# posgraph/coupe.DVSG

Hardware: AMD Instinct MI355X
Metric: stabilized frames/sec (1280x720 RGB) (higher is better)
Workload: dtype f32

## Files before the change

### coupe/dvsg_amd/_lib.py

```python
import ctypes
import os

_HERE = os.path.dirname(os.path.abspath(__file__))
LIB_PATH = os.environ.get("DVSG_AMD_LIB") or os.path.join(_HERE, "libdvsg_amd.so")
ABI_VERSION = 1

c_float_p = ctypes.POINTER(ctypes.c_float)
_vp = ctypes.c_void_p
_i = ctypes.c_int

SIGNATURES = {
    "dvsg_tps_solve_f32": [_vp, _vp, _i, _i, _i, _vp, _vp],
    "dvsg_tps_solve_checked_f32": [_vp, _vp, _i, _i, _i, _vp, _vp, _vp],
    "dvsg_tps_warp_f32": [_vp, _vp, _vp, _i, _i, _i, _i, _i, _i, _i, _vp, _vp, _vp, _vp],
    "dvsg_flow_warp_f32": [_vp, _vp, _i, _i, _i, _i, _vp, _vp],
    "dvsg_stn_sample_f32": [_vp, _vp, _vp, _i, _i, _i, _i, _i, _i, _vp, _vp],
    "dvsg_grid_affine_f32": [_vp, _vp, _i, _i, _i, _i, _i, _i, _vp, _vp, _vp, _vp],
    "dvsg_grid_projective_f32": [_vp, _vp, _i, _i, _i, _i, _i, _i, _vp, _vp, _vp, _vp],
    "dvsg_elastic_constants_f32": [_i, _vp, _vp],
    "dvsg_grid_elastic_f32": [_vp, _vp, _vp, _i, _vp, _i, _i, _i, _i, _i, _i, _vp, _vp, _vp, _vp],
    "dvsg_scale_rgb_f32": [_vp, _i, _i, _i, _i, _vp, _vp],
    "dvsg_locnet_create": [_i, ctypes.POINTER(ctypes.c_char_p), ctypes.POINTER(_vp),
                           ctypes.POINTER(_i), ctypes.POINTER(ctypes.c_int64), ctypes.POINTER(_vp)],
    "dvsg_locnet_destroy": [_vp],
# ... 99 lines not shown


def load():
    global _lib
    if _lib is not None:
        return _lib
    if not os.path.isfile(LIB_PATH):
        raise DvsgError(
            "libdvsg_amd.so not found at %s: build it with ./build.sh (hipcc --offload-arch=gfx950). "
            "coupe.dvsg_amd has no CPU or PyTorch fallback." % LIB_PATH)
    lib = ctypes.CDLL(LIB_PATH)
    lib.dvsg_abi_version.restype = ctypes.c_int
    lib.dvsg_last_error_string.restype = ctypes.c_char_p
    lib.dvsg_target_arch.restype = ctypes.c_char_p
    if lib.dvsg_abi_version() != ABI_VERSION:
        raise DvsgError("libdvsg_amd.so ABI %d != expected %d" % (lib.dvsg_abi_version(), ABI_VERSION))
    for name, argtypes in SIGNATURES.items():
        fn = getattr(lib, name)
        fn.argtypes = argtypes
        fn.restype = ctypes.c_int
    _lib = lib
    for env, opt in (("DVSG_CONV_VARIANT", b"conv_variant"), ("DVSG_FUSE_CONV", b"fuse_conv"),
                     ("DVSG_F16_SPLIT", b"f16_split"), ("DVSG_FUSE_SHORTCUT", b"fuse_shortcut"),
                     ("DVSG_CONV1_VARIANT", b"conv1_variant"), ("DVSG_F16_PAIR_MASK", b"f16_pair_mask"),
                     ("DVSG_WIDE16_PACKED", b"wide16_packed"), ("DVSG_WIDE16_AROWS", b"wide16_arows"),
                     ("DVSG_WIDE16_HREUSE", b"wide16_hreuse"), ("DVSG_FUSED_HREUSE", b"fused_hreuse"),
                     ("DVSG_CONCAT_SC", b"concat_sc"), ("DVSG_FLOW_TILED", b"flow_tiled")):
        if os.environ.get(env) and os.environ.get("DVSG_DEBUG") == "1":
            check(lib.dvsg_debug_set_option(opt, int(os.environ[env])), "dvsg_debug_set_option")
    return lib


def check(status, what):
    if status != 0:
        msg = load().dvsg_last_error_string().decode("utf-8", "replace")
        raise DvsgError("%s failed (status %d): %s" % (what, status, msg))


def call(name, *args):
    check(getattr(load(), name)(*args), name)
```

### coupe/dvsg_amd/csrc/cnn_kernels.h

```cpp
#pragma once
#include <type_traits>

#include "common.h"

namespace dvsg {

enum Precision { kF32 = 0, kF16 = 1, kF32S = 2, kF32X = 3 };
constexpr size_t elem_size(int prec) { return prec == kF16 ? 2 : 4; }
enum ConvMath { kMathF32, kMathF32S, kMathF32X, kMathF16Pairs, kMathF16Plain };
constexpr Precision storage_of(ConvMath m) { return m == kMathF32S ? kF32S : m == kMathF16Pairs || m == kMathF16Plain ? kF16 : kF32; }
constexpr ConvMath math_of(int prec, bool pairs) {
  return prec == kF16 ? (pairs ? kMathF16Pairs : kMathF16Plain) : prec == kF32S ? kMathF32S : prec == kF32X ? kMathF32X : kMathF32;
}
constexpr size_t elem_size(ConvMath m) { return elem_size((int)storage_of(m)); }
static_assert(storage_of(kMathF32) == kF32 && storage_of(kMathF32X) == kF32 && storage_of(kMathF32S) == kF32S &&
              storage_of(kMathF16Pairs) == kF16 && storage_of(kMathF16Plain) == kF16, "ConvMath -> storage format");
static_assert(math_of(kF32, false) == kMathF32 && math_of(kF32, true) == kMathF32 && math_of(kF32S, false) == kMathF32S &&
              math_of(kF32S, true) == kMathF32S && math_of(kF32X, false) == kMathF32X && math_of(kF32X, true) == kMathF32X &&
              math_of(kF16, true) == kMathF16Pairs && math_of(kF16, false) == kMathF16Plain, "(Precision, pairs) -> ConvMath");
static_assert(elem_size(kMathF32) == 4 && elem_size(kMathF32S) == 4 && elem_size(kMathF32X) == 4 &&
              elem_size(kMathF16Pairs) == 2 && elem_size(kMathF16Plain) == 2, "ConvMath -> bytes per tensor element");

struct ConvWeights {
  const void *rows = nullptr, *packed = nullptr, *packed_a = nullptr, *packed_h = nullptr;
// ... 90 lines not shown
constexpr int kSrcAligned = 1;
constexpr int kSrcKindShift = 1;
constexpr int kSrcMasked = 8;
constexpr int conv1_src(int kind, bool aligned, bool masked) {
  return (kind << kSrcKindShift) | (aligned ? kSrcAligned : 0) | (masked ? kSrcMasked : 0);
}
struct Conv1Src {
  const void *base;
  const int *table;
  int n_pool;
  const float *mask = nullptr;
};
struct Conv1Weights {
  const float *f32;
  const _Float16 *f16;
  const _Float16 *pieces;
  const unsigned short *x3;
  const float *bias;
};
int launch_conv1(int out_prec, const Conv1Src &src, int src_kind, const Conv1Weights &wt, void *y, int B, int H, int W, int Ho,
                 int Wo, int cin, hipStream_t s);
int prepare_rootconv();
int prepare_root_band();

int launch_maxpool(int prec, const void *x, void *y, int B, int H, int W, int C, int Ho, int Wo, int pad_top,
                   int pad_left, hipStream_t s);

constexpr int kPoolSplits = 8;
int launch_avgpool_partial(int prec, const void *x, float *part, int B, int HW, int C, hipStream_t s);

int launch_f16_to_f32(const void *x, float *y, size_t n, hipStream_t s);
int launch_p_to_f32(const void *x, float *y, size_t n, hipStream_t s);
int launch_f32_to_p(const float *x, void *y, size_t n, hipStream_t s);

constexpr int kDenseSplits = 8;
int launch_dense(const float *xin, int s_in, const float *bias_in, float scale_in, int lrelu_in,
                 const float *W, float *out_part, int B, int K, int N, hipStream_t s);
int launch_dense_finalize(const float *part, int s_in, float scale, const float *bias, float *out, int B,
                          int N, hipStream_t s);

}
```

### coupe/dvsg_amd/csrc/common.h

```cpp
#pragma once
#include <hip/hip_runtime.h>

#include <cstdarg>
#include <cstdio>

#include "../../../include/dvsg_amd.h"

namespace dvsg {

char *error_buffer();
int fail(int status, const char *fmt, ...) __attribute__((format(printf, 2, 3)));

inline hipStream_t as_stream(void *s) { return reinterpret_cast<hipStream_t>(s); }

inline int check_launch(const char *what) {
  hipError_t e = hipGetLastError();
  if (e != hipSuccess) return fail(DVSG_ERR_HIP, "%s: %s", what, hipGetErrorString(e));
  return DVSG_OK;
}

#define DVSG_REQUIRE(cond, ...)                                  \
  do {                                                           \
    if (!(cond)) return ::dvsg::fail(DVSG_ERR_INVALID_ARG, __VA_ARGS__); \
  } while (0)
// ... 26 lines not shown
int tps_render_impl(const double *winv_cols, const float *coord, const float *F_t, const uint8_t *src, int B, int H, int W,
                    int P, int channel_flip, float *T, float *out_f32, uint8_t *out_u8, int u8_W, int u8_x0, void *stream,
                    const float *zoom = nullptr, int render_filter = DVSG_RENDER_BILINEAR ,
                    int render_border = DVSG_BORDER_BLACK ,
                    RenderShape shape = RenderShape() );
int tps_render_nv12_check(const float *F_t, const uint8_t *y, const uint8_t *uv, size_t pitch, size_t frame_stride, int n,
                          int H, int W, const float *T, const uint8_t *out_y, const uint8_t *out_uv, size_t out_pitch,
                          size_t out_frame_stride, const char *fn = "dvsg_tps_render_nv12");
int tps_render_p010_check(const uint8_t *y, const uint8_t *uv, size_t pitch, size_t frame_stride, int n, int W,
                          const uint8_t *out_y, const uint8_t *out_uv, size_t out_pitch, size_t out_frame_stride, const char *fn);
int tps_render_nv12_impl(const double *winv_cols, const float *coord, const float *F_t, const uint8_t *y, const uint8_t *uv,
                         size_t pitch, size_t frame_stride, int n, int H, int W, int P, float *T, uint8_t *out_y,
                         uint8_t *out_uv, size_t out_pitch, size_t out_frame_stride, void *stream,
                         const float *zoom = nullptr, int render_filter = DVSG_RENDER_BILINEAR,
                         int render_border = DVSG_BORDER_BLACK, RenderShape shape = RenderShape(),
                         int surface_format = DVSG_SURFACE_NV12);
int tps_coverage_impl(const char *fn, const float *coord, long coord_bstride, const float *T, const float *zoom, int B, int P,
                      int src_H, int src_W, int out_h, int out_w, int32_t *n_border, int32_t *key_min, void *workspace,
                      size_t workspace_bytes, void *stream);

struct DebugOptions {
  int conv_variant = 0;
  int conv1_variant = 0;
  int wide16_min_tiles = 128;
  int wide16_packed = 1;
  int wide16_arows = 1;
  int wide16_hreuse = 1;
  int fused_hreuse = 1;
  int fuse_conv = 1;
  int fuse_shortcut = 1;
  int concat_sc = 1;
  int x3_conv1 = 1;
  int x3_fuse = 3;
  int f16_split = 1;
  int f16_pair_mask = 0xFFFF;
  int flow_tiled = 1;
  int flow_rounds = 4;
  int warp_xcd = 0;
};
extern DebugOptions g_opt;

inline int ceil_div(long a, long b) { return (int)((a + b - 1) / b); }

__device__ __forceinline__ uint8_t to_u8(double x) {
  const double d = x * 255.0;
  return d >= 255.0 ? (uint8_t)255 : (d > 0.0 ? (uint8_t)(int)d : (uint8_t)0);
// ... 36 lines not shown
```

### coupe/dvsg_amd/csrc/conv1_pool.hip

```cpp
#include <cstdint>
#include <type_traits>
#include <utility>

#include "cnn_device.h"
#include "cnn_kernels.h"

namespace dvsg {
namespace {

constexpr int C1_TILE = 128;
constexpr int C1_SEG_PAD = 5488;
constexpr int C1_WELEMS = 64 * kConv1Ld;
constexpr int C1_LDC = 68;

template <int NT, int GROUPS, bool ALIGNED, bool MASKED = false>
struct Conv1Row {
  static constexpr bool kRing = false;
  typedef float floatx4_u __attribute__((ext_vector_type(4), aligned(4)));
  floatx4 nmean[GROUPS];
  long idx[GROUPS];
  unsigned col_ok, full;
  bool fast;
  struct Data {
    floatx4 reg[GROUPS];
// ... 448 lines not shown
  __syncthreads();
  TO *yrow = y + (((size_t)b * Ho + ho) * Wo + wo0) * 64 + 4 * (tid & 15);
  conv1_tile_out<NT / 16>(Cs, conv1_tile_bias(bias, tid), tid, wo0, Wo,
                          [&](int row, float4 v) __attribute__((always_inline)) { store4(yrow + (size_t)row * 64, v); });
#ifdef DVSG_STAMPS
  if (tid == 0 && blockIdx.x < 65536) {
    unsigned long long *o = g_c1_stamps + (size_t)blockIdx.x * 8;
    const unsigned long long t_end = C1_STAMP();
    o[0] = st[0]; o[1] = st[1]; o[2] = st[2]; o[3] = st[3]; o[4] = st[4];
    o[5] = t_loop_end - t_begin;
    o[6] = t_end - t_begin;
    o[7] = __builtin_amdgcn_s_memrealtime() - r_begin;
  }
#endif
}

constexpr int RB_NT = 512;
constexpr int RB_IN4 = (C1_SEG_PAD / 4 + RB_NT - 1) / RB_NT;
constexpr int RB_WLOADS = (C1_WELEMS / 4 + RB_NT - 1) / RB_NT;
constexpr int RB_SLOTS = 3;
constexpr size_t RB_LDS = sizeof(float) * (size_t)(2 * C1_WELEMS + RB_SLOTS * C1_SEG_PAD);
static_assert(RB_LDS <= 160 * 1024, "the band kernel's LDS must fit a CU");

template <int SRC>
__global__ __launch_bounds__(RB_NT) __attribute__((amdgpu_waves_per_eu(2, 2)))
void root_band_kernel(const Conv1Src src, const float *__restrict__ wt1, const float *__restrict__ bias,
                      float *__restrict__ y, int H, int W, int Ho, int Wo, int wtiles, int bands, int ppb, int nbig) {
  constexpr int NT = RB_NT, MI = 2;
  static_assert(C1_TILE * C1_LDC <= C1_WELEMS, "epilogue tile must fit in a weight buffer");
  extern __shared__ __attribute__((aligned(16))) float rb_lds[];
  float *const w_s = rb_lds;
  float *const in_s = rb_lds + 2 * C1_WELEMS;
  const int tid = threadIdx.x;
  const int lane = tid & 63, wave = tid >> 6;
  const int wr = wave >> 2, wm = (wave >> 1) & 1, wn = wave & 1;
  const int r = lane & 31, h = lane >> 5;

  const Conv1Tile tile = conv1_tile(wtiles, bands);
  const int b = tile.b, band = tile.ho, wo0 = tile.wo0;
  const int pairs = (Ho + 1) / 2;
  const int p0 = band * ppb - (band > nbig ? band - nbig : 0);
  const int p1 = min(p0 + (band < nbig ? ppb : ppb - 1), pairs);
  if (p0 >= p1) return;

#ifdef DVSG_STAMPS
  unsigned long long st[8] = {0, 0, 0, 0, 0, 0, 0, 0};
  const unsigned long long t_begin = C1_STAMP(), r_begin = __builtin_amdgcn_s_memrealtime();
#endif
  typedef typename Conv1RowSel<NT, RB_IN4, SRC>::type Row;
  Row row;
  row.init(src, tid, b, wo0, H, W, C1_SEG_PAD);
  if constexpr (Row::kRing) {
    for (int e = tid; e < RB_SLOTS * C1_SEG_PAD; e += NT) in_s[e] = 0.f;
    __syncthreads();
  }
  typename Row::Data rd[3];
  floatx4 w_reg[RB_WLOADS];
  auto load_w = [&](int kh) __attribute__((always_inline)) {
    const floatx4 *wsrc = reinterpret_cast<const floatx4 *>(wt1 + (size_t)kh * C1_WELEMS);
#pragma unroll
    for (int i = 0; i < RB_WLOADS; ++i) {
      const int q = tid + NT * i;
      w_reg[i] = wsrc[q < C1_WELEMS / 4 ? q : 0];
    }
  };
  auto put_w = [&](int i, float *dst) __attribute__((always_inline)) {
    const int q = tid + NT * i;
    if (q < C1_WELEMS / 4) reinterpret_cast<floatx4 *>(dst)[q] = w_reg[i];
  };
  auto put_row = [&](const typename Row::Data &d, float *slot) __attribute__((always_inline)) {
    if constexpr (Row::kRing) {
      row.scatter(d, [&](int e, float v) __attribute__((always_inline)) { slot[e] = v; });
    } else {
#pragma unroll
      for (int i = 0; i < RB_IN4; ++i) {
        const int q = tid + NT * i;
        const floatx4 v = row.scaled(d, i);
        if (q < C1_SEG_PAD / 4) reinterpret_cast<floatx4 *>(slot)[q] = v;
      }
    }
  };
  auto load_first = [&](int ho_) __attribute__((always_inline)) {
#pragma unroll
    for (int i = 0; i < 3; ++i) row.load(rd[i], 2 * ho_ - 3 + i);
    load_w(0);
  };
#ifdef DVSG_STAMPS
  st[0] = C1_STAMP() - t_begin;
#endif
  load_first(2 * p0);

  for (int p = p0; p < p1; ++p) {
    const int ho = 2 * p;
#ifdef DVSG_STAMPS
    const unsigned long long f0 = C1_STAMP();
#endif
#pragma unroll
    for (int i = 0; i < RB_WLOADS; ++i) put_w(i, w_s);
#pragma unroll
    for (int i = 0; i < 3; ++i) {
      __builtin_amdgcn_sched_barrier(0);
      put_row(rd[i], in_s + i * C1_SEG_PAD);
    }
    __builtin_amdgcn_sched_barrier(0);
    floatx16 acc[MI], acc2[MI];
#pragma unroll
    for (int mi = 0; mi < MI; ++mi)
#pragma unroll
      for (int q = 0; q < 16; ++q) acc[mi][q] = acc2[mi][q] = 0.f;
#ifdef DVSG_STAMPS
    const unsigned long long f1 = C1_STAMP();
    __syncthreads();
    st[2] += f1 - f0;
    st[3] += C1_STAMP() - f1;
#else
    __syncthreads();
#endif

    int s_up = 0;
    for (int t = 0; t < 7; ++t) {
#ifdef DVSG_STAMPS
      const unsigned long long s3 = C1_STAMP();
#endif
      if (t < 6) {
        row.load(rd[0], 2 * ho + t);
        load_w(t + 1);
      }
#ifdef DVSG_STAMPS
      st[4] += C1_STAMP() - s3;
#endif
      __builtin_amdgcn_sched_barrier(0);
      const int s_lo = s_up == 0 ? 2 : s_up - 1;
      const float *a0 = in_s + (wr ? s_lo : s_up) * C1_SEG_PAD + 2 * kConv1Cin * (wm * 32 * MI + r) + 2 * h;
      const float *bp = w_s + (t & 1) * C1_WELEMS + (wn * 32 + r) * kConv1Ld + 2 * h;
      float *w_next = w_s + ((t + 1) & 1) * C1_WELEMS;
      constexpr int STEPS = kConv1Kpad / 4, PAIRS = (STEPS + 1) / 2;
      constexpr int WPUT0 = PAIRS / 2;
      float2 va[2][2][MI], vb[2][2];
      auto read_pair = [&](int slot, int g) __attribute__((always_inline)) {
#pragma unroll
        for (int j = 0; j < 2; ++j) {
          if (2 * g + j >= STEPS) break;
#pragma unroll
          for (int mi = 0; mi < MI; ++mi)
            va[slot][j][mi] = *reinterpret_cast<const float2 *>(a0 + mi * (2 * kConv1Cin * 32) + 4 * (2 * g + j));
          vb[slot][j] = *reinterpret_cast<const float2 *>(bp + 4 * (2 * g + j));
        }
      };
      read_pair(0, 0);
#pragma unroll
      for (int g = 0; g < PAIRS; ++g) {
        if (g + 1 < PAIRS) read_pair((g + 1) & 1, g + 1);
        if (g >= WPUT0 && g < WPUT0 + RB_WLOADS) put_w(g - WPUT0, w_next);
        __builtin_amdgcn_sched_barrier(0);
#pragma unroll
        for (int j = 0; j < 2; ++j) {
          if (2 * g + j >= STEPS) break;
#pragma unroll
          for (int mi = 0; mi < MI; ++mi) acc[mi] = mfma32(va[g & 1][j][mi].x, vb[g & 1][j].x, acc[mi]);
#pragma unroll
          for (int mi = 0; mi < MI; ++mi) acc2[mi] = mfma32(va[g & 1][j][mi].y, vb[g & 1][j].y, acc2[mi]);
        }
        __builtin_amdgcn_sched_barrier(0);
      }
      if (t < 6) {
#ifdef DVSG_STAMPS
        const unsigned long long s0 = C1_STAMP();
        __syncthreads();
        const unsigned long long s1 = C1_STAMP();
        put_row(rd[0], in_s + s_up * C1_SEG_PAD);
        const unsigned long long s2 = C1_STAMP();
        __syncthreads();
        st[1] += s1 - s0;
        st[2] += s2 - s1;
        st[3] += C1_STAMP() - s2;
#else
        __syncthreads();
        put_row(rd[0], in_s + s_up * C1_SEG_PAD);
        __syncthreads();
#endif
      }
      s_up = s_up == 2 ? 0 : s_up + 1;
    }

#ifdef DVSG_STAMPS
    const unsigned long long e0 = C1_STAMP();
#endif
    __syncthreads();
    float *Cs = w_s + wr * C1_WELEMS;
#pragma unroll
    for (int mi = 0; mi < MI; ++mi)
      C1_TILE_PUT(Cs, wm * 32 * MI + mi * 32, wn * 32, acc[mi][q] + acc2[mi][q]);
    __builtin_amdgcn_sched_barrier(0);
    if (p + 1 < p1) load_first(ho + 2);
    int tid_e = tid;
    asm volatile("" : "+v"(tid_e));
    const float4 b4 = conv1_tile_bias(bias, tid_e);
    __builtin_amdgcn_sched_barrier(0);
    __syncthreads();
#pragma unroll
    for (int j = 0; j < 2; ++j) {
      if (ho + j >= Ho) break;
      float *yrow = y + (((size_t)b * Ho + ho + j) * Wo + wo0) * 64 + 4 * (tid_e & 15);
      conv1_tile_out<NT / 16>(w_s + j * C1_WELEMS, b4, tid_e, wo0, Wo,
                              [&](int row_, float4 v) __attribute__((always_inline)) { store4(yrow + (size_t)row_ * 64, v); });
    }
    __syncthreads();
#ifdef DVSG_STAMPS
    st[5] += C1_STAMP() - e0;
#endif
  }
#ifdef DVSG_STAMPS
  if (tid == 0 && blockIdx.x < 65536) {
    unsigned long long *o = g_c1_stamps + (size_t)blockIdx.x * 8;
    o[0] = st[0]; o[1] = st[1]; o[2] = st[2]; o[3] = st[3]; o[4] = st[4]; o[5] = st[5];
    o[6] = C1_STAMP() - t_begin;
    o[7] = __builtin_amdgcn_s_memrealtime() - r_begin;
  }
#endif
}

struct PPieces {};

constexpr int rootconv_seg(int cin) { return C1_RING_PX * rootconv_pitch(cin) + 4; }
constexpr int rootconv_wstage(int cin) { return 64 * rootconv_ld(cin) > C1_TILE * C1_LDC ? 64 * rootconv_ld(cin) : C1_TILE * C1_LDC; }
constexpr size_t rootconv_lds_bytes(int cin) { return sizeof(float) * (size_t)(rootconv_wstage(cin) + rootconv_seg(cin)); }
static_assert(rootconv_lds_bytes(3 * kRootMaxFrames) <= 160 * 1024, "the largest window must fit one workgroup's LDS");

template <typename TO, int SRC>
__global__ __launch_bounds__(256)
void rootconv_kernel(const Conv1Src src, const float *__restrict__ wt1, const float *__restrict__ bias, void *__restrict__ y,
                     int H, int W, int Ho, int Wo, int wtiles, int cin) {
  constexpr int NT = 256, MI = 2;
  constexpr int kKind = SRC >> kSrcKindShift & 3;
  constexpr bool kMasked = (SRC & kSrcMasked) != 0;
  static_assert(SRC >= 0 && SRC < 16 && kKind <= kSrcRingU8, "no such conv1 source");
  extern __shared__ __attribute__((aligned(16))) float rc_lds[];
  const int S = cin / 3, pitch = rootconv_pitch(cin), ldw = rootconv_ld(cin), steps = rootconv_kpad(cin) / 4;
  const int welems = 64 * ldw, seg = rootconv_seg(cin);
  float *w_s = rc_lds;
  float *in_s = rc_lds + rootconv_wstage(cin);
  const int tid = threadIdx.x;
// ... 1228 lines not shown
int prepare_rootconv() {
  const int bytes = (int)rootconv_lds_bytes(3 * kRootMaxFrames);
  hipError_t err = hipSuccess;
  auto raise = [&](const void *fn) {
    const hipError_t e = hipFuncSetAttribute(fn, hipFuncAttributeMaxDynamicSharedMemorySize, bytes);
    if (err == hipSuccess) err = e;
  };
  for (int src = 0; src < 16; ++src)
    with_conv1_src<true>(src, [&](auto src_c) {
      constexpr int S = decltype(src_c)::value;
      raise(reinterpret_cast<const void *>(&rootconv_kernel<float, S>));
      raise(reinterpret_cast<const void *>(&rootconv_kernel<_Float16, S>));
      raise(reinterpret_cast<const void *>(&rootconv_kernel<PPieces, S>));
    });
  DVSG_HIP(err);
  return DVSG_OK;
}

int prepare_root_band() {
  hipError_t err = hipSuccess;
  for (int src = 0; src < 16; ++src)
    with_conv1_src<false>(src, [&](auto src_c) {
      constexpr int S = decltype(src_c)::value;
      const hipError_t e = hipFuncSetAttribute(reinterpret_cast<const void *>(&root_band_kernel<S>),
                                               hipFuncAttributeMaxDynamicSharedMemorySize, (int)RB_LDS);
      if (err == hipSuccess) err = e;
    });
  DVSG_HIP(err);
  return DVSG_OK;
}

#ifdef DVSG_STAMPS
extern "C" int dvsg_debug_read_conv1_stamps(void *host, size_t bytes) {
  return hipMemcpyFromSymbol(host, HIP_SYMBOL(g_c1_stamps), bytes) == hipSuccess ? 0 : -3;
}
#endif

int launch_maxpool(int prec, const void *x, void *y, int B, int H, int W, int C, int Ho, int Wo, int pad_top,
                   int pad_left, hipStream_t s) {
  DVSG_REQUIRE(C % 4 == 0 && (prec != kF32S || C % 32 == 0), "maxpool: C=%d must be a multiple of 4 (32 in the f32s format)", C);
  const size_t total = (size_t)B * Ho * Wo * (C / 4);
  const size_t want = (total + 255) / 256;
  DVSG_REQUIRE(want < (1u << 31), "maxpool: %zu blocks do not fit a grid", want);
  const int blocks = (int)want;
  ProfScope prof(kClsMaxpool, s, 0.0, (double)elem_size(prec) * C * ((double)B * H * W + (double)B * Ho * Wo));
  g_last_root_kernel[kRootMaxpool] = prec == kF32S ? 3 : (prec == kF16 ? (C % 8 == 0 ? 2 : 1) : 0);
  if (prec == kF32S)
    hipLaunchKernelGGL(maxpool_p_kernel, dim3(blocks), dim3(256), 0, s, x, y, H, W, C / 4, Ho, Wo, pad_top, pad_left, total);
  else if (prec == kF16 && C % 8 == 0) {
    const size_t total8 = total / 2;
    hipLaunchKernelGGL(maxpool_h8_kernel, dim3((unsigned)((total8 + 255) / 256)), dim3(256), 0, s, static_cast<const _Float16 *>(x),
                       static_cast<_Float16 *>(y), H, W, C / 8, Ho, Wo, pad_top, pad_left, total8);
// ... 11 lines not shown
```

### coupe/dvsg_amd/csrc/locnet.hip

```cpp
#include <atomic>
#include <cmath>
#include <cstring>
#include <map>
#include <string>
#include <vector>

#include "cnn_kernels.h"

namespace dvsg {
namespace {

constexpr float kBnEps = 1e-5f;
const char *kPrefix = "stabNet/localizationNet/";

struct HostArray {
  const float *data;
  int nd;
  int64_t dims[4];
  size_t size() const {
    size_t n = 1;
    for (int i = 0; i < nd; ++i) n *= (size_t)dims[i];
    return n;
  }
};
// ... 420 lines not shown
    } else if (act == kF32S) {
      if (int rc = launch_p_to_f32(x, act_out, n, s)) return rc;
    } else {
      DVSG_HIP(hipMemcpyAsync(act_out, x, n * sizeof(float), hipMemcpyDeviceToDevice, s));
    }
    act_dims[0] = h; act_dims[1] = w; act_dims[2] = c;
    return 1;
  };
#define DVSG_TAP(stage, x, h, w, c)            \
  do {                                         \
    int t_ = tap(stage, x, h, w, c);           \
    if (t_ < 0) return t_;                     \
    if (t_ > 0) return DVSG_OK;                \
  } while (0)
#define DVSG_RUN(call)             \
  do {                             \
    if (int rc_ = (call)) return rc_; \
  } while (0)

  DVSG_RUN(launch_zero_tickets(ws.splitk_counters, (size_t)kMaxConvLaunches * kSplitKMaxTiles, s));
  ConvScratch scratch{ws};
  const bool fuse_allowed = g_opt.fuse_conv != 0 && calib == nullptr;
  reset_root_kernel();
  {
  MarkerRange mr("dvsg/conv1");
  DVSG_RUN(launch_conv1(precision == kF32X && g_opt.x3_conv1 ? kF32X : act, src, src_kind, net->conv1.conv1_images(), ws.bufA, B, H, W,
                        d.H1, d.W1, net->c_in, s));
  }
  DVSG_TAP(0, ws.bufA, d.H1, d.W1, 64);
  {
  MarkerRange mr("dvsg/pool1");
  DVSG_RUN(launch_maxpool(act, ws.bufA, ws.bufB, B, d.H1, d.W1, 64, d.Hp, d.Wp, d.pad_top, d.pad_left, s));
  }
  DVSG_TAP(1, ws.bufB, d.Hp, d.Wp, 64);

  char *X = ws.bufB, *Y = ws.bufA;
  int h = d.Hp, w = d.Wp;
  int stage = 2;
  int unit_in_block = 0, last_block = -1;
  for (const Unit &u : net->units) {
    unit_in_block = u.block == last_block ? unit_in_block + 1 : 1;
    last_block = u.block;
    char range_name[40];
    std::snprintf(range_name, sizeof(range_name), "dvsg/block%d/unit_%d", u.block + 1, unit_in_block);
    MarkerRange mr(range_name);
    const int ho = (h - 1) / u.stride + 1, wo = (w - 1) / u.stride + 1;
    ConvRes res{X, h, w, u.stride};
    auto math = [&](int kind) { return math_of(precision, f16_pairs(net, u.block, kind)); };
    const int calib_slot = 3 * (stage - 2);
    DVSG_RUN(calib_record(calib, calib_slot, X, (long)B * h * w, u.c1.cin, s));
    const bool x3_fused = precision == kF32X && g_opt.x3_fuse == 3;
    const bool x3_unfused = precision == kF32X && (g_opt.x3_fuse == 0 || (g_opt.x3_fuse == 1 && !u.has_shortcut));
    const bool fuse23 = fuse_allowed && !x3_unfused && conv_fusable(act, u.c2.cin, u.c2.cout, u.c3.cout, u.c2.ksize) &&
                        (act != kF16 || (f16_pairs(net, u.block, kKindC2) && f16_pairs(net, u.block, kKindC3) &&
                                         (!u.has_shortcut || f16_pairs(net, u.block, kKindSc))));
// ... 189 lines not shown
  f.B = B; f.H = H; f.W = W; f.Cin = Cin; f.Cout = Cout;
  f.Ho = (H - 1) / stride + 1; f.Wo = (W - 1) / stride + 1;
  f.stride = stride;
  f.res_H = (f.Ho - 1) * res_stride + 1; f.res_W = (f.Wo - 1) * res_stride + 1; f.res_stride = res_stride;
  if (sc_x) {
    f.res = nullptr;
    f.sc_x = sc_x; f.sc_wt = sc_wt; f.sc_bias = sc_bias;
    f.sc_cin = sc_cin;
  }
  return launch_conv3x3_1x1(f, as_stream(stream));
}

int opt_any(int v) { return v; }
int opt_flag(int v) { return v != 0; }
int opt_positive(int v) { return v > 0 ? v : 1; }
int opt_mask16(int v) { return v & 0xFFFF; }
constexpr struct {
  const char *name;
  int DebugOptions::*member;
  int (*normalise)(int);
} kDebugOptions[] = {
    {"conv_variant", &DebugOptions::conv_variant, opt_any},
    {"conv1_variant", &DebugOptions::conv1_variant, opt_any},
    {"wide16_min_tiles", &DebugOptions::wide16_min_tiles, opt_any},
    {"wide16_packed", &DebugOptions::wide16_packed, opt_any},
    {"wide16_arows", &DebugOptions::wide16_arows, opt_any},
    {"wide16_hreuse", &DebugOptions::wide16_hreuse, opt_any},
    {"fused_hreuse", &DebugOptions::fused_hreuse, opt_any},
    {"fuse_conv", &DebugOptions::fuse_conv, opt_any},
    {"fuse_shortcut", &DebugOptions::fuse_shortcut, opt_flag},
    {"concat_sc", &DebugOptions::concat_sc, opt_flag},
    {"x3_conv1", &DebugOptions::x3_conv1, opt_any},
    {"x3_fuse", &DebugOptions::x3_fuse, opt_any},
    {"f16_split", &DebugOptions::f16_split, opt_flag},
    {"f16_pair_mask", &DebugOptions::f16_pair_mask, opt_mask16},
    {"flow_tiled", &DebugOptions::flow_tiled, opt_any},
    {"flow_rounds", &DebugOptions::flow_rounds, opt_positive},
    {"warp_xcd", &DebugOptions::warp_xcd, opt_flag},
};

}
}

extern "C" {

int dvsg_locnet_create(int n_arrays, const char *const *names, const float *const *host_data, const int *ndims,
// ... 652 lines not shown
```

Before: 753.2.

## Fuse root conv1 with 3x3/s2 maxpool in band kernel, fix seams separately

Adds a pooled variant of the root band conv kernel that applies bias+ReLU and a 3x3 stride-2 max-pool in the epilogue. Each block carries the previous row pair in LDS and writes pooled output directly. Partial maxima at tile and band boundaries go to a seam buffer, and a small follow-up kernel merges them. This avoids writing and re-reading the full-resolution 64-channel conv1 activation and drops the separate maxpool pass. The cost is extra LDS, seam traffic and one more launch. It only applies to the f32, even-size, unmasked case.

After: 759.9, median of 6. No clear change (+0.9%).

```diff
diff --git a/coupe/dvsg_amd/_lib.py b/coupe/dvsg_amd/_lib.py
--- a/coupe/dvsg_amd/_lib.py
+++ b/coupe/dvsg_amd/_lib.py
@@ -145,7 +145,8 @@
     _lib = lib
     for env, opt in (("DVSG_CONV_VARIANT", b"conv_variant"), ("DVSG_FUSE_CONV", b"fuse_conv"),
                      ("DVSG_F16_SPLIT", b"f16_split"), ("DVSG_FUSE_SHORTCUT", b"fuse_shortcut"),
-                     ("DVSG_CONV1_VARIANT", b"conv1_variant"), ("DVSG_F16_PAIR_MASK", b"f16_pair_mask"),
+                     ("DVSG_CONV1_VARIANT", b"conv1_variant"), ("DVSG_ROOT_POOL", b"root_pool"),
+                     ("DVSG_F16_PAIR_MASK", b"f16_pair_mask"),
                      ("DVSG_WIDE16_PACKED", b"wide16_packed"), ("DVSG_WIDE16_AROWS", b"wide16_arows"),
                      ("DVSG_WIDE16_HREUSE", b"wide16_hreuse"), ("DVSG_FUSED_HREUSE", b"fused_hreuse"),
                      ("DVSG_CONCAT_SC", b"concat_sc"), ("DVSG_FLOW_TILED", b"flow_tiled")):
diff --git a/coupe/dvsg_amd/csrc/cnn_kernels.h b/coupe/dvsg_amd/csrc/cnn_kernels.h
--- a/coupe/dvsg_amd/csrc/cnn_kernels.h
+++ b/coupe/dvsg_amd/csrc/cnn_kernels.h
@@ -136,6 +136,10 @@
                  int Wo, int cin, hipStream_t s);
 int prepare_rootconv();
 int prepare_root_band();
+bool root_pool_selected(int out_prec, const Conv1Src &src, int B, int Ho, int Wo, int cin);
+int launch_conv1_pooled(const Conv1Src &src, int src_kind, const Conv1Weights &wt, float *pooled, float *seam, int B, int H,
+                        int W, int Ho, int Wo, hipStream_t s);
+int launch_root_pool_seam(float *pooled, const float *seam, int B, int Ho, int Wo, hipStream_t s);
 
 int launch_maxpool(int prec, const void *x, void *y, int B, int H, int W, int C, int Ho, int Wo, int pad_top,
                    int pad_left, hipStream_t s);
diff --git a/coupe/dvsg_amd/csrc/common.h b/coupe/dvsg_amd/csrc/common.h
--- a/coupe/dvsg_amd/csrc/common.h
+++ b/coupe/dvsg_amd/csrc/common.h
@@ -72,6 +72,7 @@
 struct DebugOptions {
   int conv_variant = 0;
   int conv1_variant = 0;
+  int root_pool = 0;
   int wide16_min_tiles = 128;
   int wide16_packed = 1;
   int wide16_arows = 1;
diff --git a/coupe/dvsg_amd/csrc/conv1_pool.hip b/coupe/dvsg_amd/csrc/conv1_pool.hip
--- a/coupe/dvsg_amd/csrc/conv1_pool.hip
+++ b/coupe/dvsg_amd/csrc/conv1_pool.hip
@@ -494,202 +494,80 @@
 constexpr size_t RB_LDS = sizeof(float) * (size_t)(2 * C1_WELEMS + RB_SLOTS * C1_SEG_PAD);
 static_assert(RB_LDS <= 160 * 1024, "the band kernel's LDS must fit a CU");
 
+constexpr int RB_CARRY = (C1_TILE / 2) * 64;
+constexpr size_t RB_POOL_LDS = RB_LDS + sizeof(float) * (size_t)RB_CARRY;
+static_assert(RB_POOL_LDS <= 160 * 1024, "the pooled band kernel's LDS must fit a CU");
+__host__ __device__ constexpr size_t root_pool_colseam_floats(int B, int Ho, int wtiles) { return (size_t)B * Ho * (wtiles - 1) * 64; }
+__host__ __device__ constexpr int root_band_first(int band, int ppb, int nbig) { return band * ppb - (band > nbig ? band - nbig : 0); }
+
 template <int SRC>
 __global__ __launch_bounds__(RB_NT) __attribute__((amdgpu_waves_per_eu(2, 2)))
 void root_band_kernel(const Conv1Src src, const float *__restrict__ wt1, const float *__restrict__ bias,
                       float *__restrict__ y, int H, int W, int Ho, int Wo, int wtiles, int bands, int ppb, int nbig) {
-  constexpr int NT = RB_NT, MI = 2;
-  static_assert(C1_TILE * C1_LDC <= C1_WELEMS, "epilogue tile must fit in a weight buffer");
-  extern __shared__ __attribute__((aligned(16))) float rb_lds[];
-  float *const w_s = rb_lds;
-  float *const in_s = rb_lds + 2 * C1_WELEMS;
-  const int tid = threadIdx.x;
-  const int lane = tid & 63, wave = tid >> 6;
-  const int wr = wave >> 2, wm = (wave >> 1) & 1, wn = wave & 1;
-  const int r = lane & 31, h = lane >> 5;
-
-  const Conv1Tile tile = conv1_tile(wtiles, bands);
-  const int b = tile.b, band = tile.ho, wo0 = tile.wo0;
-  const int pairs = (Ho + 1) / 2;
-  const int p0 = band * ppb - (band > nbig ? band - nbig : 0);
-  const int p1 = min(p0 + (band < nbig ? ppb : ppb - 1), pairs);
-  if (p0 >= p1) return;
-
-#ifdef DVSG_STAMPS
-  unsigned long long st[8] = {0, 0, 0, 0, 0, 0, 0, 0};
-  const unsigned long long t_begin = C1_STAMP(), r_begin = __builtin_amdgcn_s_memrealtime();
-#endif
-  typedef typename Conv1RowSel<NT, RB_IN4, SRC>::type Row;
-  Row row;
-  row.init(src, tid, b, wo0, H, W, C1_SEG_PAD);
-  if constexpr (Row::kRing) {
-    for (int e = tid; e < RB_SLOTS * C1_SEG_PAD; e += NT) in_s[e] = 0.f;
-    __syncthreads();
-  }
-  typename Row::Data rd[3];
-  floatx4 w_reg[RB_WLOADS];
-  auto load_w = [&](int kh) __attribute__((always_inline)) {
-    const floatx4 *wsrc = reinterpret_cast<const floatx4 *>(wt1 + (size_t)kh * C1_WELEMS);
-#pragma unroll
-    for (int i = 0; i < RB_WLOADS; ++i) {
-      const int q = tid + NT * i;
-      w_reg[i] = wsrc[q < C1_WELEMS / 4 ? q : 0];
-    }
+#define RB_POOL 0
+#include "root_band_body.inc"
+#undef RB_POOL
+}
+
+template <int SRC>
+__global__ __launch_bounds__(RB_NT) __attribute__((amdgpu_waves_per_eu(2, 2)))
+void root_band_pool_kernel(const Conv1Src src, const float *__restrict__ wt1, const float *__restrict__ bias,
+                           float *__restrict__ y, float *__restrict__ seam, int H, int W, int Ho, int Wo, int wtiles,
+                           int bands, int ppb, int nbig) {
+#define RB_POOL 1
+#include "root_band_body.inc"
+#undef RB_POOL
+}
+
+__global__ __launch_bounds__(256)
+void root_pool_seam_kernel(float *__restrict__ y, const float *__restrict__ seam, int B, int Ho, int Wo, int wtiles, int bands,
+                           int ppb, int nbig, size_t n_row, size_t n_col) {
+  size_t e = (size_t)blockIdx.x * 256 + threadIdx.x;
+  if (e >= n_row + n_col) return;
+  const int Hp = Ho >> 1, Wp = Wo >> 1;
+  const float *colseam = seam, *rowseam = seam + root_pool_colseam_floats(B, Ho, wtiles);
+  auto max4 = [](float4 a, const float4 c) __attribute__((always_inline)) {
+    a.x = fmaxf(a.x, c.x);
+    a.y = fmaxf(a.y, c.y);
+    a.z = fmaxf(a.z, c.z);
+    a.w = fmaxf(a.w, c.w);
+    return a;
   };
-  auto put_w = [&](int i, float *dst) __attribute__((always_inline)) {
-    const int q = tid + NT * i;
-    if (q < C1_WELEMS / 4) reinterpret_cast<floatx4 *>(dst)[q] = w_reg[i];
-  };
-  auto put_row = [&](const typename Row::Data &d, float *slot) __attribute__((always_inline)) {
-    if constexpr (Row::kRing) {
-      row.scatter(d, [&](int e, float v) __attribute__((always_inline)) { slot[e] = v; });
-    } else {
-#pragma unroll
-      for (int i = 0; i < RB_IN4; ++i) {
-        const int q = tid + NT * i;
-        const floatx4 v = row.scaled(d, i);
-        if (q < C1_SEG_PAD / 4) reinterpret_cast<floatx4 *>(slot)[q] = v;
-      }
-    }
-  };
-  auto load_first = [&](int ho_) __attribute__((always_inline)) {
-#pragma unroll
-    for (int i = 0; i < 3; ++i) row.load(rd[i], 2 * ho_ - 3 + i);
-    load_w(0);
-  };
-#ifdef DVSG_STAMPS
-  st[0] = C1_STAMP() - t_begin;
-#endif
-  load_first(2 * p0);
-
-  for (int p = p0; p < p1; ++p) {
-    const int ho = 2 * p;
-#ifdef DVSG_STAMPS
-    const unsigned long long f0 = C1_STAMP();
-#endif
-#pragma unroll
-    for (int i = 0; i < RB_WLOADS; ++i) put_w(i, w_s);
+  int c4, pc, pr, t = -1;
+  size_t b;
+  float4 m;
+  if (e < n_row) {
+    c4 = (int)(e % 16);
+    e /= 16;
+    pc = (int)(e % Wp);
+    e /= Wp;
+    const int k = (int)(e % (bands - 1));
+    b = e / (bands - 1);
+    pr = root_band_first(k + 1, ppb, nbig) - 1;
+    m = load4(y + (((b * Hp + pr) * Wp + pc) * 64 + 4 * c4));
+    m = max4(m, load4(rowseam + (((b * (bands - 1) + k) * Wp + pc) * 64 + 4 * c4)));
+    if (pc % (C1_TILE / 2) == C1_TILE / 2 - 1 && pc + 1 < Wp) t = pc / (C1_TILE / 2);
+  } else {
+    e -= n_row;
+    c4 = (int)(e % 16);
+    e /= 16;
+    t = (int)(e % (wtiles - 1));
+    e /= wtiles - 1;
+    pr = (int)(e % Hp);
+    b = e / Hp;
+    pc = (C1_TILE / 2) * (t + 1) - 1;
+    const int band = pr < nbig * ppb ? pr / ppb : nbig + (pr - nbig * ppb) / (ppb > 1 ? ppb - 1 : 1);
+    if (band + 1 < bands && root_band_first(band + 1, ppb, nbig) == pr + 1) return;
+    m = load4(y + (((b * Hp + pr) * Wp + pc) * 64 + 4 * c4));
+  }
+  if (t >= 0) {
 #pragma unroll
     for (int i = 0; i < 3; ++i) {
-      __builtin_amdgcn_sched_barrier(0);
-      put_row(rd[i], in_s + i * C1_SEG_PAD);
-    }
-    __builtin_amdgcn_sched_barrier(0);
-    floatx16 acc[MI], acc2[MI];
-#pragma unroll
-    for (int mi = 0; mi < MI; ++mi)
-#pragma unroll
-      for (int q = 0; q < 16; ++q) acc[mi][q] = acc2[mi][q] = 0.f;
-#ifdef DVSG_STAMPS
-    const unsigned long long f1 = C1_STAMP();
-    __syncthreads();
-    st[2] += f1 - f0;
-    st[3] += C1_STAMP() - f1;
-#else
-    __syncthreads();
-#endif
-
-    int s_up = 0;
-    for (int t = 0; t < 7; ++t) {
-#ifdef DVSG_STAMPS
-      const unsigned long long s3 = C1_STAMP();
-#endif
-      if (t < 6) {
-        row.load(rd[0], 2 * ho + t);
-        load_w(t + 1);
-      }
-#ifdef DVSG_STAMPS
-      st[4] += C1_STAMP() - s3;
-#endif
-      __builtin_amdgcn_sched_barrier(0);
-      const int s_lo = s_up == 0 ? 2 : s_up - 1;
-      const float *a0 = in_s + (wr ? s_lo : s_up) * C1_SEG_PAD + 2 * kConv1Cin * (wm * 32 * MI + r) + 2 * h;
-      const float *bp = w_s + (t & 1) * C1_WELEMS + (wn * 32 + r) * kConv1Ld + 2 * h;
-      float *w_next = w_s + ((t + 1) & 1) * C1_WELEMS;
-      constexpr int STEPS = kConv1Kpad / 4, PAIRS = (STEPS + 1) / 2;
-      constexpr int WPUT0 = PAIRS / 2;
-      float2 va[2][2][MI], vb[2][2];
-      auto read_pair = [&](int slot, int g) __attribute__((always_inline)) {
-#pragma unroll
-        for (int j = 0; j < 2; ++j) {
-          if (2 * g + j >= STEPS) break;
-#pragma unroll
-          for (int mi = 0; mi < MI; ++mi)
-            va[slot][j][mi] = *reinterpret_cast<const float2 *>(a0 + mi * (2 * kConv1Cin * 32) + 4 * (2 * g + j));
-          vb[slot][j] = *reinterpret_cast<const float2 *>(bp + 4 * (2 * g + j));
-        }
-      };
-      read_pair(0, 0);
-#pragma unroll
-      for (int g = 0; g < PAIRS; ++g) {
-        if (g + 1 < PAIRS) read_pair((g + 1) & 1, g + 1);
-        if (g >= WPUT0 && g < WPUT0 + RB_WLOADS) put_w(g - WPUT0, w_next);
-        __builtin_amdgcn_sched_barrier(0);
-#pragma unroll
-        for (int j = 0; j < 2; ++j) {
-          if (2 * g + j >= STEPS) break;
-#pragma unroll
-          for (int mi = 0; mi < MI; ++mi) acc[mi] = mfma32(va[g & 1][j][mi].x, vb[g & 1][j].x, acc[mi]);
-#pragma unroll
-          for (int mi = 0; mi < MI; ++mi) acc2[mi] = mfma32(va[g & 1][j][mi].y, vb[g & 1][j].y, acc2[mi]);
-        }
-        __builtin_amdgcn_sched_barrier(0);
-      }
-      if (t < 6) {
-#ifdef DVSG_STAMPS
-        const unsigned long long s0 = C1_STAMP();
-        __syncthreads();
-        const unsigned long long s1 = C1_STAMP();
-        put_row(rd[0], in_s + s_up * C1_SEG_PAD);
-        const unsigned long long s2 = C1_STAMP();
-        __syncthreads();
-        st[1] += s1 - s0;
-        st[2] += s2 - s1;
-        st[3] += C1_STAMP() - s2;
-#else
-        __syncthreads();
-        put_row(rd[0], in_s + s_up * C1_SEG_PAD);
-        __syncthreads();
-#endif
-      }
-      s_up = s_up == 2 ? 0 : s_up + 1;
-    }
-
-#ifdef DVSG_STAMPS
-    const unsigned long long e0 = C1_STAMP();
-#endif
-    __syncthreads();
-    float *Cs = w_s + wr * C1_WELEMS;
-#pragma unroll
-    for (int mi = 0; mi < MI; ++mi)
-      C1_TILE_PUT(Cs, wm * 32 * MI + mi * 32, wn * 32, acc[mi][q] + acc2[mi][q]);
-    __builtin_amdgcn_sched_barrier(0);
-    if (p + 1 < p1) load_first(ho + 2);
-    int tid_e = tid;
-    asm volatile("" : "+v"(tid_e));
-    const float4 b4 = conv1_tile_bias(bias, tid_e);
-    __builtin_amdgcn_sched_barrier(0);
-    __syncthreads();
-#pragma unroll
-    for (int j = 0; j < 2; ++j) {
-      if (ho + j >= Ho) break;
-      float *yrow = y + (((size_t)b * Ho + ho + j) * Wo + wo0) * 64 + 4 * (tid_e & 15);
-      conv1_tile_out<NT / 16>(w_s + j * C1_WELEMS, b4, tid_e, wo0, Wo,
-                              [&](int row_, float4 v) __attribute__((always_inline)) { store4(yrow + (size_t)row_ * 64, v); });
-    }
-    __syncthreads();
-#ifdef DVSG_STAMPS
-    st[5] += C1_STAMP() - e0;
-#endif
-  }
-#ifdef DVSG_STAMPS
-  if (tid == 0 && blockIdx.x < 65536) {
-    unsigned long long *o = g_c1_stamps + (size_t)blockIdx.x * 8;
-    o[0] = st[0]; o[1] = st[1]; o[2] = st[2]; o[3] = st[3]; o[4] = st[4]; o[5] = st[5];
-    o[6] = C1_STAMP() - t_begin;
-    o[7] = __builtin_amdgcn_s_memrealtime() - r_begin;
-  }
-#endif
+      const int hi = 2 * pr + i;
+      if (hi < Ho) m = max4(m, load4(colseam + (((b * Ho + hi) * (wtiles - 1) + t) * 64 + 4 * c4)));
+    }
+  }
+  store4(y + (((b * Hp + pr) * Wp + pc) * 64 + 4 * c4), m);
 }
 
 struct PPieces {};
@@ -1964,12 +1842,74 @@
   for (int src = 0; src < 16; ++src)
     with_conv1_src<false>(src, [&](auto src_c) {
       constexpr int S = decltype(src_c)::value;
-      const hipError_t e = hipFuncSetAttribute(reinterpret_cast<const void *>(&root_band_kernel<S>),
-                                               hipFuncAttributeMaxDynamicSharedMemorySize, (int)RB_LDS);
+      hipError_t e = hipFuncSetAttribute(reinterpret_cast<const void *>(&root_band_kernel<S>),
+                                         hipFuncAttributeMaxDynamicSharedMemorySize, (int)RB_LDS);
+      if (err == hipSuccess) err = e;
+      e = hipFuncSetAttribute(reinterpret_cast<const void *>(&root_band_pool_kernel<S>),
+                              hipFuncAttributeMaxDynamicSharedMemorySize, (int)RB_POOL_LDS);
       if (err == hipSuccess) err = e;
     });
   DVSG_HIP(err);
   return DVSG_OK;
+}
+
+namespace {
+bool root_band_plan(int B, int Ho, int wtiles, int *bands, int *ppb, int *nbig) {
+  const int variant = g_opt.conv1_variant;
+  *bands = variant == 0 || variant == 6 ? root_bands(B, Ho, wtiles, ppb, nbig) : 0;
+  if (variant == 6) {
+    *ppb = 3;
+    *bands = *nbig = ((Ho + 1) / 2 + *ppb - 1) / *ppb;
+  }
+  return *bands > 0;
+}
+}
+
+bool root_pool_selected(int out_prec, const Conv1Src &src, int B, int Ho, int Wo, int cin) {
+  int bands, ppb, nbig;
+  return out_prec == kF32 && cin == kConv1Cin && !src.mask && g_opt.root_pool == 0 && Ho % 2 == 0 && Wo % 2 == 0 &&
+         root_band_plan(B, Ho, ceil_div(Wo, C1_TILE), &bands, &ppb, &nbig);
+}
+
+int launch_conv1_pooled(const Conv1Src &src, int src_kind, const Conv1Weights &wt, float *pooled, float *seam, int B, int H,
+                        int W, int Ho, int Wo, hipStream_t s) {
+  DVSG_REQUIRE(root_pool_selected(kF32, src, B, Ho, Wo, kConv1Cin) && wt.f32, "conv1 + pool: not a launch of the pooled band kernel");
+  const int wtiles = ceil_div(Wo, C1_TILE);
+  int bands, ppb, nbig;
+  root_band_plan(B, Ho, wtiles, &bands, &ppb, &nbig);
+  const long blocks = (long)wtiles * bands * B;
+  DVSG_REQUIRE(blocks > 0 && blocks < (1L << 31), "conv1: grid of %ld workgroups out of range", blocks);
+  DVSG_REQUIRE((long)W * kConv1Cin < (1L << 31), "conv1: input row too long");
+  DVSG_REQUIRE(src_kind == kSrcWindow || (src.table && src.n_pool > 0), "conv1: a frame ring needs its index table");
+  const double in_bytes = src_kind == kSrcRingU8 ? 1.0 : 4.0;
+  ProfScope prof(kClsConv1, s, 2.0 * (double)B * Ho * Wo * 64 * 49 * kConv1Cin,
+                 in_bytes * (double)B * H * W * kConv1Cin +
+                     4.0 * 64 * B * ((double)(Ho / 2) * (Wo / 2) + (double)Ho * (wtiles - 1) + (double)(bands - 1) * (Wo / 2)));
+  const bool aligned = W % 4 == 0 && reinterpret_cast<uintptr_t>(src.base) % (src_kind == kSrcRingU8 ? 4 : 16) == 0;
+  const int SRC = conv1_src(src_kind, aligned, false);
+  const bool legal = with_conv1_src<false>(SRC, [&](auto src_c) {
+    constexpr int S = decltype(src_c)::value;
+    record_conv1_kernel(7, 8, 0, S, bands, ppb);
+    hipLaunchKernelGGL((root_band_pool_kernel<S>), dim3((unsigned)blocks), dim3(RB_NT), RB_POOL_LDS, s, src, wt.f32, wt.bias, pooled,
+                       seam, H, W, Ho, Wo, wtiles, bands, ppb, nbig);
+  });
+  DVSG_REQUIRE(legal, "conv1: no kernel for source %d", SRC);
+  return check_launch("root_band_pool_kernel");
+}
+
+int launch_root_pool_seam(float *pooled, const float *seam, int B, int Ho, int Wo, hipStream_t s) {
+  const int wtiles = ceil_div(Wo, C1_TILE);
+  int bands, ppb, nbig;
+  DVSG_REQUIRE(Ho % 2 == 0 && Wo % 2 == 0 && root_band_plan(B, Ho, wtiles, &bands, &ppb, &nbig), "pool seams: not the pooled path");
+  g_last_root_kernel[kRootMaxpool] = 4;
+  const size_t n_row = (size_t)B * (bands - 1) * (Wo / 2) * 16, n_col = (size_t)B * (Ho / 2) * (wtiles - 1) * 16;
+  if (n_row + n_col == 0) return DVSG_OK;
+  const size_t want = (n_row + n_col + 255) / 256;
+  DVSG_REQUIRE(want < (1u << 31), "pool seams: %zu blocks do not fit a grid", want);
+  ProfScope prof(kClsMaxpool, s, 0.0, 16.0 * (3.0 * (double)n_row + 5.0 * (double)n_col));
+  hipLaunchKernelGGL(root_pool_seam_kernel, dim3((unsigned)want), dim3(256), 0, s, pooled, seam, B, Ho, Wo, wtiles, bands, ppb, nbig,
+                     n_row, n_col);
+  return check_launch("root_pool_seam_kernel");
 }
 
 #ifdef DVSG_STAMPS
diff --git a/coupe/dvsg_amd/csrc/locnet.hip b/coupe/dvsg_amd/csrc/locnet.hip
--- a/coupe/dvsg_amd/csrc/locnet.hip
+++ b/coupe/dvsg_amd/csrc/locnet.hip
@@ -466,15 +466,25 @@
   ConvScratch scratch{ws};
   const bool fuse_allowed = g_opt.fuse_conv != 0 && calib == nullptr;
   reset_root_kernel();
+  const int conv1_prec = precision == kF32X && g_opt.x3_conv1 ? kF32X : act;
+  if (stop_stage != 0 && root_pool_selected(conv1_prec, src, B, d.H1, d.W1, net->c_in)) {
+    {
+    MarkerRange mr("dvsg/conv1");
+    DVSG_RUN(launch_conv1_pooled(src, src_kind, net->conv1.conv1_images(), reinterpret_cast<float *>(ws.bufB),
+                                 reinterpret_cast<float *>(ws.bufA), B, H, W, d.H1, d.W1, s));
+    }
+    MarkerRange mr("dvsg/pool1");
+    DVSG_RUN(launch_root_pool_seam(reinterpret_cast<float *>(ws.bufB), reinterpret_cast<const float *>(ws.bufA), B, d.H1, d.W1, s));
+  } else {
   {
   MarkerRange mr("dvsg/conv1");
-  DVSG_RUN(launch_conv1(precision == kF32X && g_opt.x3_conv1 ? kF32X : act, src, src_kind, net->conv1.conv1_images(), ws.bufA, B, H, W,
-                        d.H1, d.W1, net->c_in, s));
+  DVSG_RUN(launch_conv1(conv1_prec, src, src_kind, net->conv1.conv1_images(), ws.bufA, B, H, W, d.H1, d.W1, net->c_in, s));
   }
   DVSG_TAP(0, ws.bufA, d.H1, d.W1, 64);
   {
   MarkerRange mr("dvsg/pool1");
   DVSG_RUN(launch_maxpool(act, ws.bufA, ws.bufB, B, d.H1, d.W1, 64, d.Hp, d.Wp, d.pad_top, d.pad_left, s));
+  }
   }
   DVSG_TAP(1, ws.bufB, d.Hp, d.Wp, 64);
 
@@ -710,6 +720,7 @@
 } kDebugOptions[] = {
     {"conv_variant", &DebugOptions::conv_variant, opt_any},
     {"conv1_variant", &DebugOptions::conv1_variant, opt_any},
+    {"root_pool", &DebugOptions::root_pool, opt_any},
     {"wide16_min_tiles", &DebugOptions::wide16_min_tiles, opt_any},
     {"wide16_packed", &DebugOptions::wide16_packed, opt_any},
     {"wide16_arows", &DebugOptions::wide16_arows, opt_any},
diff --git a/coupe/dvsg_amd/csrc/root_band_body.inc b/coupe/dvsg_amd/csrc/root_band_body.inc
--- /dev/null
+++ b/coupe/dvsg_amd/csrc/root_band_body.inc
@@ -0,0 +1,248 @@
+  constexpr int NT = RB_NT, MI = 2;
+  static_assert(C1_TILE * C1_LDC <= C1_WELEMS, "epilogue tile must fit in a weight buffer");
+  extern __shared__ __attribute__((aligned(16))) float rb_lds[];
+  float *const w_s = rb_lds;
+  float *const in_s = rb_lds + 2 * C1_WELEMS;
+  const int tid = threadIdx.x;
+  const int lane = tid & 63, wave = tid >> 6;
+  const int wr = wave >> 2, wm = (wave >> 1) & 1, wn = wave & 1;
+  const int r = lane & 31, h = lane >> 5;
+
+  const Conv1Tile tile = conv1_tile(wtiles, bands);
+  const int b = tile.b, band = tile.ho, wo0 = tile.wo0;
+  const int pairs = (Ho + 1) / 2;
+  const int p0 = band * ppb - (band > nbig ? band - nbig : 0);
+  const int p1 = min(p0 + (band < nbig ? ppb : ppb - 1), pairs);
+  if (p0 >= p1) return;
+
+#ifdef DVSG_STAMPS
+  unsigned long long st[8] = {0, 0, 0, 0, 0, 0, 0, 0};
+  const unsigned long long t_begin = C1_STAMP(), r_begin = __builtin_amdgcn_s_memrealtime();
+#endif
+  typedef typename Conv1RowSel<NT, RB_IN4, SRC>::type Row;
+  Row row;
+  row.init(src, tid, b, wo0, H, W, C1_SEG_PAD);
+  if constexpr (Row::kRing) {
+    for (int e = tid; e < RB_SLOTS * C1_SEG_PAD; e += NT) in_s[e] = 0.f;
+    __syncthreads();
+  }
+  typename Row::Data rd[3];
+  floatx4 w_reg[RB_WLOADS];
+  auto load_w = [&](int kh) __attribute__((always_inline)) {
+    const floatx4 *wsrc = reinterpret_cast<const floatx4 *>(wt1 + (size_t)kh * C1_WELEMS);
+#pragma unroll
+    for (int i = 0; i < RB_WLOADS; ++i) {
+      const int q = tid + NT * i;
+      w_reg[i] = wsrc[q < C1_WELEMS / 4 ? q : 0];
+    }
+  };
+  auto put_w = [&](int i, float *dst) __attribute__((always_inline)) {
+    const int q = tid + NT * i;
+    if (q < C1_WELEMS / 4) reinterpret_cast<floatx4 *>(dst)[q] = w_reg[i];
+  };
+  auto put_row = [&](const typename Row::Data &d, float *slot) __attribute__((always_inline)) {
+    if constexpr (Row::kRing) {
+      row.scatter(d, [&](int e, float v) __attribute__((always_inline)) { slot[e] = v; });
+    } else {
+#pragma unroll
+      for (int i = 0; i < RB_IN4; ++i) {
+        const int q = tid + NT * i;
+        const floatx4 v = row.scaled(d, i);
+        if (q < C1_SEG_PAD / 4) reinterpret_cast<floatx4 *>(slot)[q] = v;
+      }
+    }
+  };
+  auto load_first = [&](int ho_) __attribute__((always_inline)) {
+#pragma unroll
+    for (int i = 0; i < 3; ++i) row.load(rd[i], 2 * ho_ - 3 + i);
+    load_w(0);
+  };
+#ifdef DVSG_STAMPS
+  st[0] = C1_STAMP() - t_begin;
+#endif
+  load_first(2 * p0);
+
+  for (int p = p0; p < p1; ++p) {
+    const int ho = 2 * p;
+#ifdef DVSG_STAMPS
+    const unsigned long long f0 = C1_STAMP();
+#endif
+#pragma unroll
+    for (int i = 0; i < RB_WLOADS; ++i) put_w(i, w_s);
+#pragma unroll
+    for (int i = 0; i < 3; ++i) {
+      __builtin_amdgcn_sched_barrier(0);
+      put_row(rd[i], in_s + i * C1_SEG_PAD);
+    }
+    __builtin_amdgcn_sched_barrier(0);
+    floatx16 acc[MI], acc2[MI];
+#pragma unroll
+    for (int mi = 0; mi < MI; ++mi)
+#pragma unroll
+      for (int q = 0; q < 16; ++q) acc[mi][q] = acc2[mi][q] = 0.f;
+#ifdef DVSG_STAMPS
+    const unsigned long long f1 = C1_STAMP();
+    __syncthreads();
+    st[2] += f1 - f0;
+    st[3] += C1_STAMP() - f1;
+#else
+    __syncthreads();
+#endif
+
+    int s_up = 0;
+    for (int t = 0; t < 7; ++t) {
+#ifdef DVSG_STAMPS
+      const unsigned long long s3 = C1_STAMP();
+#endif
+      if (t < 6) {
+        row.load(rd[0], 2 * ho + t);
+        load_w(t + 1);
+      }
+#ifdef DVSG_STAMPS
+      st[4] += C1_STAMP() - s3;
+#endif
+      __builtin_amdgcn_sched_barrier(0);
+      const int s_lo = s_up == 0 ? 2 : s_up - 1;
+      const float *a0 = in_s + (wr ? s_lo : s_up) * C1_SEG_PAD + 2 * kConv1Cin * (wm * 32 * MI + r) + 2 * h;
+      const float *bp = w_s + (t & 1) * C1_WELEMS + (wn * 32 + r) * kConv1Ld + 2 * h;
+      float *w_next = w_s + ((t + 1) & 1) * C1_WELEMS;
+      constexpr int STEPS = kConv1Kpad / 4, PAIRS = (STEPS + 1) / 2;
+      constexpr int WPUT0 = PAIRS / 2;
+      float2 va[2][2][MI], vb[2][2];
+      auto read_pair = [&](int slot, int g) __attribute__((always_inline)) {
+#pragma unroll
+        for (int j = 0; j < 2; ++j) {
+          if (2 * g + j >= STEPS) break;
+#pragma unroll
+          for (int mi = 0; mi < MI; ++mi)
+            va[slot][j][mi] = *reinterpret_cast<const float2 *>(a0 + mi * (2 * kConv1Cin * 32) + 4 * (2 * g + j));
+          vb[slot][j] = *reinterpret_cast<const float2 *>(bp + 4 * (2 * g + j));
+        }
+      };
+      read_pair(0, 0);
+#pragma unroll
+      for (int g = 0; g < PAIRS; ++g) {
+        if (g + 1 < PAIRS) read_pair((g + 1) & 1, g + 1);
+        if (g >= WPUT0 && g < WPUT0 + RB_WLOADS) put_w(g - WPUT0, w_next);
+        __builtin_amdgcn_sched_barrier(0);
+#pragma unroll
+        for (int j = 0; j < 2; ++j) {
+          if (2 * g + j >= STEPS) break;
+#pragma unroll
+          for (int mi = 0; mi < MI; ++mi) acc[mi] = mfma32(va[g & 1][j][mi].x, vb[g & 1][j].x, acc[mi]);
+#pragma unroll
+          for (int mi = 0; mi < MI; ++mi) acc2[mi] = mfma32(va[g & 1][j][mi].y, vb[g & 1][j].y, acc2[mi]);
+        }
+        __builtin_amdgcn_sched_barrier(0);
+      }
+      if (t < 6) {
+#ifdef DVSG_STAMPS
+        const unsigned long long s0 = C1_STAMP();
+        __syncthreads();
+        const unsigned long long s1 = C1_STAMP();
+        put_row(rd[0], in_s + s_up * C1_SEG_PAD);
+        const unsigned long long s2 = C1_STAMP();
+        __syncthreads();
+        st[1] += s1 - s0;
+        st[2] += s2 - s1;
+        st[3] += C1_STAMP() - s2;
+#else
+        __syncthreads();
+        put_row(rd[0], in_s + s_up * C1_SEG_PAD);
+        __syncthreads();
+#endif
+      }
+      s_up = s_up == 2 ? 0 : s_up + 1;
+    }
+
+#ifdef DVSG_STAMPS
+    const unsigned long long e0 = C1_STAMP();
+#endif
+    __syncthreads();
+    float *Cs = w_s + wr * C1_WELEMS;
+#pragma unroll
+    for (int mi = 0; mi < MI; ++mi)
+      C1_TILE_PUT(Cs, wm * 32 * MI + mi * 32, wn * 32, acc[mi][q] + acc2[mi][q]);
+    __builtin_amdgcn_sched_barrier(0);
+    if (p + 1 < p1) load_first(ho + 2);
+    int tid_e = tid;
+    asm volatile("" : "+v"(tid_e));
+    const float4 b4 = conv1_tile_bias(bias, tid_e);
+    __builtin_amdgcn_sched_barrier(0);
+    __syncthreads();
+#if RB_POOL
+    {
+      const int Wp = Wo >> 1;
+      const float *Cs4 = w_s + 4 * (tid_e & 15);
+      auto at = [&](int j, int col) __attribute__((always_inline)) {
+        float4 v = *reinterpret_cast<const float4 *>(Cs4 + j * C1_WELEMS + col * C1_LDC);
+        v.x = fmaxf(v.x + b4.x, 0.f);
+        v.y = fmaxf(v.y + b4.y, 0.f);
+        v.z = fmaxf(v.z + b4.z, 0.f);
+        v.w = fmaxf(v.w + b4.w, 0.f);
+        return v;
+      };
+      auto max4 = [](float4 a, const float4 c) __attribute__((always_inline)) {
+        a.x = fmaxf(a.x, c.x);
+        a.y = fmaxf(a.y, c.y);
+        a.z = fmaxf(a.z, c.z);
+        a.w = fmaxf(a.w, c.w);
+        return a;
+      };
+      if (wo0 > 0 && tid_e < 32) {
+        const int j = tid_e >> 4;
+        store4(seam + (((size_t)b * Ho + ho + j) * (wtiles - 1) + (wo0 / C1_TILE - 1)) * 64 + 4 * (tid_e & 15), at(j, 0));
+      }
+#pragma unroll
+      for (int k = 0; k < 2; ++k) {
+        const int c = (tid_e >> 4) + 32 * k;
+        if (wo0 + 2 * c >= Wo) break;
+        const bool third = 2 * c + 2 < C1_TILE && wo0 + 2 * c + 2 < Wo;
+        float4 u = max4(at(0, 2 * c), at(0, 2 * c + 1)), l = max4(at(1, 2 * c), at(1, 2 * c + 1));
+        if (third) {
+          u = max4(u, at(0, 2 * c + 2));
+          l = max4(l, at(1, 2 * c + 2));
+        }
+        float4 *cr = reinterpret_cast<float4 *>(in_s + RB_SLOTS * C1_SEG_PAD + c * 64 + 4 * (tid_e & 15));
+        const size_t pc = (size_t)(wo0 >> 1) + c;
+        if (p > p0)
+          store4(y + ((((size_t)b * (Ho >> 1) + p - 1) * Wp + pc) * 64 + 4 * (tid_e & 15)), max4(*cr, u));
+        else if (band > 0)
+          store4(seam + root_pool_colseam_floats(gridDim.x / (wtiles * bands), Ho, wtiles) +
+                     ((((size_t)b * (bands - 1) + band - 1) * Wp + pc) * 64 + 4 * (tid_e & 15)), u);
+        *cr = max4(u, l);
+      }
+    }
+#else
+#pragma unroll
+    for (int j = 0; j < 2; ++j) {
+      if (ho + j >= Ho) break;
+      float *yrow = y + (((size_t)b * Ho + ho + j) * Wo + wo0) * 64 + 4 * (tid_e & 15);
+      conv1_tile_out<NT / 16>(w_s + j * C1_WELEMS, b4, tid_e, wo0, Wo,
+                              [&](int row_, float4 v) __attribute__((always_inline)) { store4(yrow + (size_t)row_ * 64, v); });
+    }
+#endif
+    __syncthreads();
+#ifdef DVSG_STAMPS
+    st[5] += C1_STAMP() - e0;
+#endif
+  }
+#if RB_POOL
+  {
+#pragma unroll
+    for (int k = 0; k < 2; ++k) {
+      const int c = (tid >> 4) + 32 * k;
+      if (wo0 + 2 * c >= Wo) break;
+      const float4 m = *reinterpret_cast<const float4 *>(in_s + RB_SLOTS * C1_SEG_PAD + c * 64 + 4 * (tid & 15));
+      store4(y + ((((size_t)b * (Ho >> 1) + p1 - 1) * (Wo >> 1) + (wo0 >> 1) + c) * 64 + 4 * (tid & 15)), m);
+    }
+  }
+#endif
+#ifdef DVSG_STAMPS
+  if (tid == 0 && blockIdx.x < 65536) {
+    unsigned long long *o = g_c1_stamps + (size_t)blockIdx.x * 8;
+    o[0] = st[0]; o[1] = st[1]; o[2] = st[2]; o[3] = st[3]; o[4] = st[4]; o[5] = st[5];
+    o[6] = C1_STAMP() - t_begin;
+    o[7] = __builtin_amdgcn_s_memrealtime() - r_begin;
+  }
+#endif
```
